# MAC-VO/MAC-VO

Hardware: AMD Instinct MI355X
Metric: stereo frames/sec at 640x480 (hot path: cost volume + lookup, keypoint selection, covariance, PGO) (higher is better)
Workload: dtype f32 via f16x2 (volume: fp32 operands row-scaled by powers of two and split into two fp16 pieces, three products, fp32 accumulate, scales undone exactly) + f32 (lookup/covariance) + f64 (PGO)

## Files before the change

mac-vo_amd/csrc/frontend_ops.hip:

```cpp
#include "common.h"
#include "randperm_dev.h"
#include "kp_draw_dev.h"
#include "match_cov_dev.h"
#include "pose_apply_dev.h"
#include "obs_filter_dev.h"
#include <math.h>

namespace {

__global__ __launch_bounds__(256) void frontend_epilogue_kernel(
    const float* __restrict__ flow, const float* __restrict__ logcov, int cov_is_log, int plane, float bl_fx,
    float bl_fx_sq, float* __restrict__ disparity, float* __restrict__ disparity_cov, float* __restrict__ depth,
    float* __restrict__ depth_cov, uint8_t* __restrict__ bad_mask, float* __restrict__ match_flow,
    float* __restrict__ match_cov) {
    MV_CHAIN_KERNEL_PRIO();
    const size_t lo = (size_t)blockIdx.y * plane;
    flow += 4 * lo; logcov += 4 * lo;
    if (disparity) disparity += lo;
    if (disparity_cov) disparity_cov += lo;
    if (depth) depth += lo;
    if (depth_cov) depth_cov += lo;
    if (bad_mask) bad_mask += lo;
    if (match_flow) match_flow += 2 * lo;
    if (match_cov) match_cov += 3 * lo;
// ... 224 lines not shown
    if (out_sdd) out_sdd[n] = depth_cov ? depth_cov[i] : -1.f;
    if (out_sigma) { out_sigma[3 * n] = match_cov_default; out_sigma[3 * n + 1] = match_cov_default; out_sigma[3 * n + 2] = 0.f; }
    const float pc[3] = {d, ((uf - cx) * d) / fx, ((vf - cy) * d) / fy};
    if (out_Tc) { out_Tc[3 * n] = pc[0]; out_Tc[3 * n + 1] = pc[1]; out_Tc[3 * n + 2] = pc[2]; }
    if (out_Tw) {
        const float q[4] = {pose[3], pose[4], pose[5], pose[6]};
        float r[3];
        quat_act_f32(q, pc, r);
        out_Tw[3 * n] = r[0] + pose[0]; out_Tw[3 * n + 1] = r[1] + pose[1]; out_Tw[3 * n + 2] = r[2] + pose[2];
    }
    if (out_color && image) {
        const size_t plane = (size_t)H * W;
#pragma unroll
        for (int c = 0; c < 3; ++c) {
            const float x = image[c * plane + i] * 255.f;
            out_color[3 * n + c] = (uint8_t)(int)x;
        }
    }
}

__global__ __launch_bounds__(256) void obs_filter_kernel(const uint8_t* __restrict__ inbound,
                                                         const double* __restrict__ cov1,
                                                         const double* __restrict__ cov2,
                                                         const float* __restrict__ vals, int flags,
                                                         float min_depth, float max_depth, int cap, mvLaneCounts cnt,
                                                         uint8_t* __restrict__ valid, int32_t* __restrict__ count) {
    obs_filter_body(inbound, cov1, cov2, vals, flags, min_depth, max_depth, cap, cnt.n[blockIdx.x], blockIdx.x, gridDim.x, valid, count);
}

struct DrawArgs {
    const int32_t* count;
    int count_stride;
    float nomatch_c;
    const uint32_t* state_in;
    uint32_t* state_out;
    int k;
    int32_t cov_mods;
    int64_t* out_perm;
    int32_t* out_live;
};
struct DrawLds {
    mvrp::Scratch s;
    int32_t head[mvrp::NBUCKET];
    int32_t out[mvrp::MAX_HEAD];
};
template <int PM, int MODEL = MV_COV_MATCH, bool MODS = false, bool NOMATCH = false>
__global__ __launch_bounds__(256) void backend_front_kernel(const int32_t* __restrict__ cand, size_t cand_lane_stride, const int64_t* __restrict__ perm,
                                                            PermArg pa, int cap, mvLaneCounts cnt, int64_t* out_uv, TrackArgs a, float fx, float fy,
                                                            float cx, float cy, float* pos_Tc, const float* depth_map0, const float* depth_map1,
                                                            double* out_cov0, double* out_cov1, mvMatchCovParams cp, DrawArgs da) {
    __shared__ __attribute__((aligned(16))) char draw_raw[PM == 2 ? sizeof(DrawLds) : PM == 4 ? sizeof(mvkp::Scratch) : 16];
    DrawLds& D = *reinterpret_cast<DrawLds*>(draw_raw);
    const int lane = threadIdx.x & 63;
    const int n = blockIdx.x * 4 + (threadIdx.x >> 6);
    const int set = blockIdx.y, pl = blockIdx.z;
    int N;
    if constexpr (PM == 2) {
        const int64_t n_cand = da.count[(size_t)pl * da.count_stride];
        const bool adv = blockIdx.x == 0 && blockIdx.y == 0;
        N = mv_randperm_head_wg(da.state_in + (size_t)pl * mvrp::MT_STRIDE, adv ? da.state_out + (size_t)pl * mvrp::MT_STRIDE : nullptr, n_cand, da.k,
                                D.out, D.s, D.head);
        __syncthreads();
        if (adv) {
            for (int i = threadIdx.x; i < N; i += 256) da.out_perm[(size_t)pl * cap + i] = D.out[i];
            if (threadIdx.x == 0) { da.out_live[2 * pl] = N; da.out_live[2 * pl + 1] = (int32_t)n_cand; }
        }
    } else if constexpr (PM == 3) {
        if (da.count) {
            const int c = da.count[(size_t)pl * da.count_stride];
            N = c < 0 ? 0 : (c > cap ? cap : c);
        } else {
            N = cnt.n[pl];
        }
        if (da.out_live && blockIdx.x == 0 && blockIdx.y == 0 && threadIdx.x == 0) { da.out_live[2 * pl] = N; da.out_live[2 * pl + 1] = N; }
    } else if constexpr (PM == 4) {
        N = cnt.n[pl];
        const bool adv = blockIdx.x == 0 && blockIdx.y == 0;
        mv_kp_random_wg(da.state_in + (size_t)pl * mvrp::MT_STRIDE, adv ? da.state_out + (size_t)pl * mvrp::MT_STRIDE : nullptr, da.k,
                        *reinterpret_cast<mvkp::Scratch*>(draw_raw));
    } else {
        N = cnt.n[pl];
    }
    if (n < N) {
        int u0, v0;
        if constexpr (PM <= 2) {
            const int32_t* cand_l = cand + (size_t)pl * cand_lane_stride;
            const long pi = PM == 2 ? (long)D.out[n] : PM == 1 ? (long)pa.idx[n] : (long)perm[(size_t)pl * cap + n];
            const int lin = cand_l[pi];
            u0 = lin % a.W;
            v0 = lin / a.W;
        } else if constexpr (PM == 3) {
            const int64_t* kp = perm + 2 * ((size_t)pl * cap + n);
            u0 = (int)kp[0];
            v0 = (int)kp[1];
        } else if constexpr (PM == 4) {
            mvkp::row_of(reinterpret_cast<mvkp::Scratch*>(draw_raw)->w, da.k, n, a.H, a.W, pa.idx[0], u0, v0);
        } else {
            mvkp::grid_row(mvkp::Grid{pa.idx[0], 0, pa.idx[1], pa.idx[2], pa.idx[3]}, n, u0, v0);
        }
        TrackArgs al = a;
        track_lane_offsets(al, pl, cap);
        const size_t ln = (size_t)pl * cap;
        float u, v, suu, svv, suv;
        if (set == 0) {
            if (lane == 0) {
                if (PM != 3 || out_uv != perm) {
                    out_uv[2 * (ln + n) + 0] = u0;
                    out_uv[2 * (ln + n) + 1] = v0;
                }
                kp_track_one(n, u0, v0, al.match_flow, al.match_cov, al.depth0, al.disp0, al.sdisp0, al.sdd0, al.depth1, al.disp1, al.sdisp1, al.sdd1,
                             al.H, al.W, al.edge, al.match_cov_default, al.out_kp0, al.out_kp1, al.out_inbound, al.out_vals, (size_t)gridDim.z * cap,
                             nullptr, nullptr);
                al.out_sigma0[3 * n + 2] = 0.f;
                const float uf = (float)u0, vf = (float)v0, d = al.out_vals[n];
                float* pt = pos_Tc + 3 * (ln + n);
                pt[0] = d;
                pt[1] = ((uf - cx) * d) / fx;
                pt[2] = ((vf - cy) * d) / fy;
// ... 178 lines not shown
}

int mv_backend_front(const mvKpSource& src, int lanes, int cap, const mvFrontMaps& m, const mvCovConfig& cv, const mvFrontTables& t, mvStream_t stream) {
    const mvMatchCovParams& cp = cv.cp;
    const int kind = src.kind, num_point = src.num_point;
    MV_CHECK_ARG(kind >= MV_KPSRC_PERM && kind <= MV_KPSRC_GRID && cv.edge >= 0);
    if (kind != MV_KPSRC_PERM) MV_CHECK_ARG(lanes >= 1 && lanes <= MV_MAX_LANES && cap >= 1 && num_point >= 0);
    if (kind == MV_KPSRC_DRAW) MV_CHECK_ARG(num_point <= cap && src.n_live_stride >= 1);
    if (kind >= MV_KPSRC_ROWS) MV_CHECK_ARG(src.mask_width >= 0);
    MV_CHECK_ARG(cv.model >= MV_COV_MATCH && cv.model <= MV_COV_NONE && mv_cov_modifiers_ok(cv.modifiers));
    MV_CHECK_ARG(cv.model != MV_COV_GMM || (m.f0.sdd && m.f1.sdd));
    const bool nomatch = (cv.nocov & MV_NOCOV_MATCH) != 0;
    MV_CHECK_ARG(!nomatch || (m.match_cov == nullptr && kind >= MV_KPSRC_ROWS));
    MV_CHECK_ARG(!(cv.nocov & MV_NOCOV_DEPTH) || (cv.model != MV_COV_GMM && !m.f0.sdd && !m.f1.sdd && !m.f0.sdisp && !m.f1.sdisp));
    MV_CHECK_ARG(cp.H > 0 && cp.W > 0 && cp.kernel_size >= 1 && (cp.kernel_size & 1) && cp.use_patch_var);
    if (cp.kernel_size > mvcov::MAX_K || (kind == MV_KPSRC_DRAW && num_point > mvrp::MAX_HEAD)) return MV_ERR_UNSUPPORTED;
    mvLaneCounts c{};
    int n_max = 0;
    if (kind == MV_KPSRC_PERM) {
        const int rc = check_lanes(lanes, src.n_live, cap, c, n_max);
        if (rc != MV_OK) return rc;
        if (n_max == 0) return MV_OK;
    }
    MV_CHECK_ARG(m.match_flow && m.f0.depth && m.f1.depth && t.kp0_uv && t.kp1 && t.inbound && t.vals && t.sigma0 && t.sigma1 && t.pos_Tc && t.cov0 &&
                 t.cov1);
    const TrackArgs ta{m.match_flow, m.match_cov, m.f0.depth, m.f0.disp, m.f0.sdisp, m.f0.sdd, m.f1.depth, m.f1.disp, m.f1.sdisp, m.f1.sdd, cp.H, cp.W,
                       cv.edge, cv.match_cov_default, t.kp0, t.kp1, t.inbound, t.vals, t.sigma0, t.sigma1};
    const int32_t* cand = nullptr;
    size_t cand_stride = 0;
    const int64_t* rows = nullptr;
    PermArg pa;
    pa.idx[0] = 0;
    DrawArgs da{};
    int pm;
    if (kind == MV_KPSRC_PERM) {
        MV_CHECK_ARG(src.cand && (src.perm_dev || src.perm_host));
        cand = src.cand;
        cand_stride = src.cand_lane_stride;
        if (src.perm_host && lanes == 1 && n_max <= 256) {
            for (int i = 0; i < n_max; ++i) {
                MV_CHECK_ARG(src.perm_host[i] >= 0 && src.perm_host[i] <= 0x7fffffffLL);
                pa.idx[i] = (int32_t)src.perm_host[i];
            }
            pm = 1;
        } else {
            MV_CHECK_ARG(src.perm_dev);
            rows = src.perm_dev;
            pm = 0;
        }
    } else if (kind == MV_KPSRC_DRAW) {
        MV_CHECK_ARG(src.cand && src.n_live_dev && src.state_in && src.state_out && src.state_in != src.state_out && src.out_perm && src.out_live);
        cand = src.cand;
        cand_stride = src.cand_lane_stride;
        n_max = num_point > 0 ? num_point : 1;
        da = DrawArgs{src.n_live_dev, src.n_live_stride, 0.f, src.state_in, src.state_out, num_point, 0, src.out_perm, src.out_live};
        pm = 2;
    } else if (kind == MV_KPSRC_ROWS) {
        MV_CHECK_ARG(src.rows && (src.n_live || (src.n_live_dev && src.n_live_stride >= 1)));
        da.out_live = src.out_live;
        if (src.n_live) {
            const int rc = check_lanes(lanes, src.n_live, cap, c, n_max);
            if (rc != MV_OK) return rc;
        } else {
            n_max = cap;
            da.count = src.n_live_dev;
            da.count_stride = src.n_live_stride;
        }
        if (n_max == 0) return MV_OK;
        rows = src.rows;
        pm = 3;
    } else if (kind == MV_KPSRC_RANDOM) {
        MV_CHECK_ARG(src.state_in && src.state_out && src.state_in != src.state_out && num_point >= 1 && num_point <= cap && cp.H > 2 * src.mask_width &&
                     cp.W > 2 * src.mask_width);
        if (num_point > mvkp::MAX_POINT) return MV_ERR_UNSUPPORTED;
        n_max = num_point;
        pa.idx[0] = src.mask_width;
        da.state_in = src.state_in;
        da.state_out = src.state_out;
        da.k = num_point;
        pm = 4;
    } else {
        mvkp::Grid g;
        n_max = mvkp::grid_of(cp.H, cp.W, src.mask_width, num_point, &g);
        MV_CHECK_ARG(n_max >= 1 && n_max <= cap);
        pa.idx[0] = g.cols; pa.idx[1] = g.sh; pa.idx[2] = g.sw; pa.idx[3] = g.mask;
        pm = 5;
    }
    if (pm >= 4)
        for (int l = 0; l < lanes; ++l) c.n[l] = n_max;
    const dim3 grid(mv_ceil_div(n_max, 4), 2, lanes);
    launch_backend_front_pm(pm, cv.model, cv.modifiers, nomatch, cv.model_match_cov_default, grid, (hipStream_t)stream, da, cand, cand_stride, rows, pa, cap, c, t.kp0_uv, ta, cp.fx, cp.fy, cp.cx,
                            cp.cy, t.pos_Tc, m.f0.depth, m.f1.depth, t.cov0, t.cov1, cp);
    return mv_launch_status();
}

extern "C" int mv_backend_front_lanes(const int32_t* cand, size_t cand_lane_stride, const int64_t* perm_dev, const int64_t* perm_host, int lanes,
                                      const int32_t* n_live, int cap, const float* match_flow, const float* match_cov, const float* depth0,
                                      const float* disp0, const float* sdisp0, const float* sdd0, const float* depth1, const float* disp1,
                                      const float* sdisp1, const float* sdd1, int edge, float match_cov_default, const mvMatchCovParams* cov_params,
                                      int64_t* out_kp0_uv, float* out_kp0, float* out_kp1, uint8_t* out_inbound, float* out_vals, float* out_sigma0,
                                      float* out_sigma1, float* out_pos_Tc, double* out_cov0, double* out_cov1, mvStream_t stream) {
    MV_CHECK_ARG(cov_params);
    mvKpSource src{};
    src.kind = MV_KPSRC_PERM;
    src.cand = cand; src.cand_lane_stride = cand_lane_stride; src.perm_dev = perm_dev; src.perm_host = perm_host; src.n_live = n_live;
    return mv_backend_front(src, lanes, cap, {match_flow, match_cov, {depth0, disp0, sdisp0, sdd0}, {depth1, disp1, sdisp1, sdd1}},
                            {MV_COV_MATCH, 0, *cov_params, edge, match_cov_default},
                            {out_kp0_uv, out_kp0, out_kp1, out_inbound, out_vals, out_sigma0, out_sigma1, out_pos_Tc, out_cov0, out_cov1}, stream);
}

extern "C" int mv_backend_front_draw_lanes(const int32_t* cand, size_t cand_lane_stride, const int32_t* count_dev, int count_stride, const uint32_t* state_in,
                                           uint32_t* state_out, int num_point, int lanes, int cap, const float* match_flow, const float* match_cov,
                                           const float* depth0, const float* disp0, const float* sdisp0, const float* sdd0, const float* depth1,
                                           const float* disp1, const float* sdisp1, const float* sdd1, int edge, float match_cov_default,
                                           const mvMatchCovParams* cov_params, int64_t* out_perm, int32_t* out_live, int64_t* out_kp0_uv, float* out_kp0,
                                           float* out_kp1, uint8_t* out_inbound, float* out_vals, float* out_sigma0, float* out_sigma1, float* out_pos_Tc,
                                           double* out_cov0, double* out_cov1, mvStream_t stream) {
    MV_CHECK_ARG(cov_params);
    mvKpSource src{};
    src.kind = MV_KPSRC_DRAW;
    src.cand = cand; src.cand_lane_stride = cand_lane_stride; src.n_live_dev = count_dev; src.n_live_stride = count_stride;
    src.state_in = state_in; src.state_out = state_out; src.num_point = num_point; src.out_perm = out_perm; src.out_live = out_live;
    return mv_backend_front(src, lanes, cap, {match_flow, match_cov, {depth0, disp0, sdisp0, sdd0}, {depth1, disp1, sdisp1, sdd1}},
                            {MV_COV_MATCH, 0, *cov_params, edge, match_cov_default},
                            {out_kp0_uv, out_kp0, out_kp1, out_inbound, out_vals, out_sigma0, out_sigma1, out_pos_Tc, out_cov0, out_cov1}, stream);
}

extern "C" int mv_kp_track(const int64_t* kp0_uv, int N, const float* match_flow, const float* match_cov,
                           const float* depth0, const float* disp0, const float* sdisp0, const float* sdd0,
                           const float* depth1, const float* disp1, const float* sdisp1, const float* sdd1, int H,
                           int W, int edge, float match_cov_default, float* out_kp0, float* out_kp1,
                           uint8_t* out_inbound, float* out_vals, float* out_sigma0, float* out_sigma1,
                           mvStream_t stream) {
    MV_CHECK_ARG(N >= 0);
    const int32_t n = N;
    return mv_kp_track_lanes(kp0_uv, 1, &n, N, match_flow, match_cov, depth0, disp0, sdisp0, sdd0, depth1, disp1, sdisp1,
                             sdd1, H, W, edge, match_cov_default, out_kp0, out_kp1, out_inbound, out_vals, out_sigma0,
                             out_sigma1, stream);
}

extern "C" int mv_backproject_lanes(const float* kp_uv, const float* depth_vals, int depth_stride, size_t depth_lane_stride,
                                    float fx, float fy, float cx, float cy, const float* pose, int lanes,
                                    const int32_t* n_live, int cap, float* pos_Tc, float* pos_Tw, double* rot,
// ... 78 lines not shown
```

mac-vo_amd/csrc/kp_select.hip:

```cpp
#include "common.h"
#include <math.h>

namespace {

#ifdef MV_KP_PROFILE
__device__ long long g_kp_stamps[16];
#define KP_STAMP(i) do { if (threadIdx.x == 0) g_kp_stamps[i] = wall_clock64(); } while (0)
#else
#define KP_STAMP(i)
#endif

constexpr int TILE_W = 64;
constexpr int TILE_H = 16;
constexpr int MAX_R = 7;
constexpr unsigned CAND_FLAG = 0x80000000u;

struct KpWs {
    unsigned long long* cand_bits;
    unsigned* rec_idx;
    float* rec_q;
    float* rec_d;
    int* counters;
    size_t lane_bytes;

    __device__ __forceinline__ KpWs lane(int l) const {
        const size_t o = (size_t)l * lane_bytes;
        return KpWs{(unsigned long long*)((char*)cand_bits + o), (unsigned*)((char*)rec_idx + o), (float*)((char*)rec_q + o),
                    (float*)((char*)rec_d + o), (int*)((char*)counters + o), lane_bytes};
    }
};

__device__ __forceinline__ float flow_quality(const float* __restrict__ fc, int plane, int idx) {
    const float c0 = fc[idx], c1 = fc[plane + idx], c2 = fc[2 * plane + idx];
    return (c0 + c1) - 2.f * c2;
}

__device__ __forceinline__ float nanmin(float a, float b) { return (a < b || a != a) ? a : b; }

template <bool FUSE>
__global__ __launch_bounds__(256) void kp_nms_kernel(const float* __restrict__ fc, const float* __restrict__ d0,
                                                      const float* __restrict__ d0c, const float* __restrict__ d1,
                                                      const float* __restrict__ d1c,
                                                      const uint8_t* __restrict__ mask_a,
                                                      const uint8_t* __restrict__ mask_b, mvKpSelectParams p,
                                                      KpWs ws_all, int words_per_row, mvEpiArgs ef) {
    MV_CHAIN_KERNEL_PRIO();
    const KpWs ws = ws_all.lane(blockIdx.z);
    {
        const size_t lp = (size_t)blockIdx.z * p.H * p.W;
        if (fc) fc += 3 * lp;
        if (d0) d0 += lp;
        if (d0c) d0c += lp;
        if (d1) d1 += lp;
        if (d1c) d1c += lp;
        if (mask_a) mask_a += lp;
        if (mask_b) mask_b += lp;
        if (FUSE) {
            ef.flow += 4 * lp; ef.logcov += 4 * lp;
            if (ef.disparity) ef.disparity += lp;
            if (ef.disparity_cov) ef.disparity_cov += lp;
            if (ef.depth) ef.depth += lp;
            if (ef.depth_cov) ef.depth_cov += lp;
            if (ef.bad_mask) ef.bad_mask += lp;
            if (ef.match_flow) ef.match_flow += 2 * lp;
            if (ef.match_cov) ef.match_cov += 3 * lp;
        }
    }
    __shared__ float tile[TILE_H + 2 * MAX_R][TILE_W + 2 * MAX_R + 1];
    __shared__ float hmin[TILE_H + 2 * MAX_R][TILE_W + 1];
    __shared__ int wg_count, wg_base;
    const int H = p.H, W = p.W, plane = H * W;
    const int r = p.kernel_size >> 1;
    const int x0 = blockIdx.x * TILE_W, y0 = blockIdx.y * TILE_H;
    const int tx = threadIdx.x, ty = threadIdx.y;
    const int tid = ty * 64 + tx;
    const bool mapping = p.mode == MV_KP_MAPPING;
    if (tid == 0) wg_count = 0;

    if (!mapping) {
        const int tw = TILE_W + 2 * r, th = TILE_H + 2 * r;
        constexpr int NST = ((TILE_W + 2 * MAX_R) * (TILE_H + 2 * MAX_R) + 255) / 256;
// ... 29 lines not shown
        for (int e = tid; e < th * TILE_W; e += 256) {
            const int ly = e >> 6, lx = e & 63;
            float m = tile[ly][lx];
            for (int dx = 1; dx <= 2 * r; ++dx) m = nanmin(m, tile[ly][lx + dx]);
            hmin[ly][lx] = m;
        }
    }
    __syncthreads();

    bool nms_px[TILE_H / 4];
    bool cand_px[TILE_H / 4];
    float q_px[TILE_H / 4];
    int my_nms = 0;
#pragma unroll
    for (int it = 0; it < TILE_H / 4; ++it) {
        const int ly = ty * (TILE_H / 4) + it;
        const int gx = x0 + tx, gy = y0 + ly;
        const bool inimg = gx < W && gy < H;
        const int idx = gy * W + gx;
        bool nms = false, cand = false;
        float q = 0.f;
        if (FUSE && inimg) mv_epilogue_pixel(ef, plane, idx);
        if (inimg) {
            const bool border = p.mask_width > 0 && gx >= p.mask_width && gx < W - p.mask_width &&
                                gy >= p.mask_width && gy < H - p.mask_width;
            if (mapping) {
                cand = border && (d0[idx] < p.max_depth) && (d0c[idx] < p.max_depth_cov);
            } else {
                q = tile[ly + r][tx + r];
                float m = hmin[ly][tx];
                for (int dy = 1; dy <= 2 * r; ++dy) m = nanmin(m, hmin[ly + dy][tx]);
                nms = (q == m);
                cand = nms && border;
                if (cand && p.mode == MV_KP_FULL) cand = (d0[idx] < p.max_depth) && (d1[idx] < p.max_depth);
            }
            if (cand && mask_a) cand = mask_a[idx] != 0;
            if (cand && mask_b) cand = mask_b[idx] != 0;
        }
        const unsigned long long cand_word = __ballot(cand);
        if (tx == 0 && gy < H) ws.cand_bits[(size_t)gy * words_per_row + blockIdx.x] = cand_word;
        nms_px[it] = nms;
        cand_px[it] = cand;
        q_px[it] = q;
        my_nms += nms;
    }
    if (mapping) return;

    int my_off = 0;
    if (my_nms) my_off = atomicAdd(&wg_count, my_nms);
    __syncthreads();
#ifdef MV_KP_FAKE_ATOMIC
    if (tid == 0) wg_base = (blockIdx.y * gridDim.x + blockIdx.x) * 16;
#else
    if (tid == 0) wg_base = wg_count ? atomicAdd(&ws.counters[0], wg_count) : 0;
#endif
    __syncthreads();
    int pos = wg_base + my_off;
#pragma unroll
    for (int it = 0; it < TILE_H / 4; ++it) {
        if (nms_px[it]) {
            const int gx = x0 + tx, gy = y0 + ty * (TILE_H / 4) + it;
            const int idx = gy * W + gx;
            ws.rec_idx[pos] = (unsigned)(((gy * words_per_row + blockIdx.x) << 6) | tx) | (cand_px[it] ? CAND_FLAG : 0u);
            if (p.mode == MV_KP_NODEPTH) {
                ws.rec_q[pos] = q_px[it];
            } else {
                ws.rec_q[pos] = fc ? flow_quality(fc, plane, idx) : 0.f;
                ws.rec_d[pos] = d0c[idx];
            }
            ++pos;
        }
    }
}

__device__ __forceinline__ unsigned float_key(float f) {
    if (f != f) return 0xFFFFFFFFu;
    const unsigned u = __float_as_uint(f);
    return (u & 0x80000000u) ? ~u : (u | 0x80000000u);
}
__device__ __forceinline__ float key_float(unsigned k) {
    const unsigned u = (k & 0x80000000u) ? (k & 0x7FFFFFFFu) : ~k;
    return __uint_as_float(u);
}

#ifndef MV_KP_FINISH_THREADS
#define MV_KP_FINISH_THREADS 1024
#endif

constexpr int RANK_CAP = 256;
constexpr unsigned NAN_KEY = 0xFFFFFFFFu;

template <int NT>
__device__ __forceinline__ int block_exclusive_scan(int v, int* wave_tot , int& total) {
    constexpr int NW = NT / 64;
    const int tid = threadIdx.x;
    int incl = v;
#pragma unroll
    for (int o = 1; o < 64; o <<= 1) {
        const int t = __shfl_up(incl, o, 64);
        if ((tid & 63) >= o) incl += t;
    }
    __syncthreads();
    if ((tid & 63) == 63) wave_tot[tid >> 6] = incl;
    __syncthreads();
    int off = 0;
    total = 0;
#pragma unroll
    for (int w = 0; w < NW; ++w) {
        const int t = wave_tot[w];
        if (w < (tid >> 6)) off += t;
        total += t;
    }
    return off + incl - v;
}

template <int NT, bool CACHED, int RPT, typename F>
__device__ __forceinline__ void for_each_key(const float* __restrict__ vals, int n, const unsigned (&keys)[RPT], F&& f) {
    const int tid = threadIdx.x;
    if (CACHED) {
        const int nr = (n + NT - 1) / NT;
#pragma unroll
        for (int r = 0; r < RPT; ++r)
            if (r < nr && r * NT + tid < n) f(keys[r]);
    } else {
        for (int i = tid; i < n; i += NT) f(float_key(vals[i]));
    }
}

struct MedianLds {
    unsigned hist[2048];
    unsigned lst[RANK_CAP];
    unsigned red_lo[16], red_hi[16];
    int red_cnt[16];
    int wave_tot[16];
    int sh[4];
    unsigned res;
};

template <int NT, bool CACHED, int RPT>
__device__ float block_nanmedian(const float* __restrict__ vals, int n, const unsigned (&keys)[RPT], MedianLds& L) {
    constexpr int NW = NT / 64, BPT = 2048 / NT;
    const int tid = threadIdx.x;
    unsigned lo = NAN_KEY, hi = 0u;
    int cnt = 0;
    for_each_key<NT, CACHED, RPT>(vals, n, keys, [&](unsigned k) {
        if (k != NAN_KEY) {
            lo = min(lo, k);
            hi = max(hi, k);
            ++cnt;
        }
    });
#pragma unroll
    for (int o = 32; o > 0; o >>= 1) {
        lo = min(lo, (unsigned)__shfl_xor((int)lo, o, 64));
        hi = max(hi, (unsigned)__shfl_xor((int)hi, o, 64));
        cnt += __shfl_xor(cnt, o, 64);
    }
    __syncthreads();
    if ((tid & 63) == 0) {
        L.red_lo[tid >> 6] = lo;
        L.red_hi[tid >> 6] = hi;
        L.red_cnt[tid >> 6] = cnt;
    }
    __syncthreads();
    cnt = 0;
#pragma unroll
    for (int w = 0; w < NW; ++w) {
        lo = min(lo, L.red_lo[w]);
        hi = max(hi, L.red_hi[w]);
        cnt += L.red_cnt[w];
    }
    if (cnt <= 0) return NAN;
    int k = (cnt - 1) >> 1;
    for (;;) {
        if (lo == hi) return key_float(lo);
        const unsigned span = hi - lo;
        const int s = max(0, 32 - __clz((int)span) - 11);
#pragma unroll
        for (int j = 0; j < BPT; ++j) L.hist[j * NT + tid] = 0;
        if (tid == 0) L.sh[3] = 0;
        __syncthreads();
        for_each_key<NT, CACHED, RPT>(vals, n, keys, [&](unsigned kk) {
            if (kk >= lo && kk <= hi) atomicAdd(&L.hist[(kk - lo) >> s], 1u);
        });
        __syncthreads();
        int c[BPT], sum = 0;
#pragma unroll
        for (int j = 0; j < BPT; ++j) {
            c[j] = (int)L.hist[tid * BPT + j];
            sum += c[j];
        }
        int total;
        const int excl = block_exclusive_scan<NT>(sum, L.wave_tot, total);
        if (excl <= k && k < excl + sum) {
            int before = excl;
#pragma unroll
            for (int j = 0; j < BPT; ++j) {
                if (k >= before && k < before + c[j]) {
                    L.sh[0] = tid * BPT + j;
                    L.sh[1] = c[j];
                    L.sh[2] = k - before;
                }
                before += c[j];
            }
        }
        __syncthreads();
        const unsigned b = (unsigned)L.sh[0];
        const int cb = L.sh[1];
        k = L.sh[2];
        const unsigned nlo = lo + (b << s);
        const unsigned w = s ? ((1u << s) - 1u) : 0u;
        const unsigned nhi = (hi - nlo < w) ? hi : nlo + w;
        if (cb <= RANK_CAP) {
            for_each_key<NT, CACHED, RPT>(vals, n, keys, [&](unsigned kk) {
                if (kk >= nlo && kk <= nhi) L.lst[atomicAdd(&L.sh[3], 1)] = kk;
            });
            __syncthreads();
            for (int i = tid; i < cb; i += NT) {
                const unsigned e = L.lst[i];
                int rank = 0;
                for (int j = 0; j < cb; ++j) {
                    const unsigned o = L.lst[j];
                    rank += (o < e) || (o == e && j < i);
                }
                if (rank == k) L.res = e;
            }
            __syncthreads();
            return key_float(L.res);
        }
        lo = nlo;
        hi = nhi;
        __syncthreads();
    }
}

template <int NT, bool FAST, int RPT, int WPT, bool USE_D>
__device__ __forceinline__ void kp_finish_body(const mvKpSelectParams& p, const KpWs& ws, int has_flow, int words_per_row,
                                               int32_t* __restrict__ out_cand, int32_t* __restrict__ out_count,
                                               float* __restrict__ out_stats, int n_rec, MedianLds& L,
                                               unsigned long long* lds_words) {
    constexpr int RD = USE_D ? RPT : 1;
    const int tid = threadIdx.x;
    const int H = p.H, W = p.W;
    const bool mapping = p.mode == MV_KP_MAPPING;
    const bool use_f = (p.mode == MV_KP_NODEPTH) || (p.mode == MV_KP_FULL && has_flow);
    const bool use_d = USE_D && (p.mode == MV_KP_FULL);
    const int n_words = H * words_per_row;

    unsigned kq[RPT], kd[RD], ridx[RPT];
    unsigned long long wreg[WPT];
    KP_STAMP(0);
    if (FAST) {
        const int cap = H * W;
#pragma unroll
        for (int r = 0; r < RPT; ++r) {
            const int i = min(r * NT + tid, cap - 1);
            ridx[r] = mapping ? 0u : ws.rec_idx[i];
            kq[r] = use_f ? __float_as_uint(ws.rec_q[i]) : 0u;
            if (USE_D) kd[r] = use_d ? __float_as_uint(ws.rec_d[i]) : 0u;
        }
#pragma unroll
        for (int j = 0; j < WPT; ++j) {
            const int w = j * NT + tid;
            wreg[j] = w < n_words ? ws.cand_bits[w] : 0ull;
        }
#pragma unroll
        for (int r = 0; r < RPT; ++r) {
            const bool live = r * NT + tid < n_rec;
            ridx[r] = live ? ridx[r] : 0u;
            kq[r] = live ? float_key(__uint_as_float(kq[r])) : NAN_KEY;
            if (USE_D) kd[r] = live ? float_key(__uint_as_float(kd[r])) : NAN_KEY;
        }
    }

    float med_f = NAN, thr_f = INFINITY, med_d = NAN, thr_d = INFINITY;
    KP_STAMP(1);
    if (use_f) {
        med_f = block_nanmedian<NT, FAST, RPT>(ws.rec_q, n_rec, kq, L);
        const float prod = med_f * 1.5f;
        thr_f = (prod < p.max_match_cov) ? prod : p.max_match_cov;
    }
    if (use_d) {
        med_d = block_nanmedian<NT, FAST, RD>(ws.rec_d, n_rec, kd, L);
        const float prod = med_d * 1.5f;
        thr_d = (prod < p.max_depth_cov) ? prod : p.max_depth_cov;
    }

    KP_STAMP(2);
    const int per = (n_words + NT - 1) / NT;
    unsigned long long cw[WPT];
    if (FAST) {
        constexpr int NPASS = WPT > 5 * 1024 / NT ? 8 : 2;
        constexpr int TPP = NT / NPASS;
        unsigned fail = 0;
        if (!mapping) {
            const int nr = (n_rec + NT - 1) / NT;
#pragma unroll
            for (int r = 0; r < RPT; ++r) {
                if (r < nr && (ridx[r] & CAND_FLAG)) {
                    bool ok = true;
                    if (use_f) ok = key_float(kq[r]) < thr_f;
                    if (USE_D) { if (ok && use_d) ok = key_float(kd[USE_D ? r : 0]) < thr_d; }
                    if (!ok) fail |= 1u << r;
                }
            }
        }
#pragma unroll
        for (int i = 0; i < WPT; ++i) cw[i] = 0ull;
#pragma unroll 1
        for (int h = 0; h < NPASS; ++h) {
            const int wlo = h * TPP * per, whi = min(wlo + TPP * per, n_words);
#pragma unroll
            for (int j = 0; j < WPT; ++j) {
                const int w = j * NT + tid;
                if (w >= wlo && w < whi) lds_words[w - wlo] = wreg[j];
            }
            __syncthreads();
            if (fail) {
#pragma unroll
                for (int r = 0; r < RPT; ++r) {
                    const int w = (int)((ridx[r] & ~CAND_FLAG) >> 6);
                    if (((fail >> r) & 1u) && w >= wlo && w < whi) atomicAnd(&lds_words[w - wlo], ~(1ull << (ridx[r] & 63)));
                }
            }
            __syncthreads();
            if (tid / TPP == h) {
#pragma unroll
                for (int i = 0; i < WPT; ++i) {
                    const int w = tid * per + i;
                    if (i < per && w < whi) cw[i] = lds_words[w - wlo];
                }
            }
            __syncthreads();
        }
    } else if (!mapping) {
        for (int i = tid; i < n_rec; i += NT) {
            const unsigned ri = ws.rec_idx[i];
            if (ri & CAND_FLAG) {
                bool ok = true;
                if (use_f) ok = ws.rec_q[i] < thr_f;
                if (ok && use_d) ok = ws.rec_d[i] < thr_d;
                if (!ok) atomicAnd(&ws.cand_bits[(ri & ~CAND_FLAG) >> 6], ~(1ull << (ri & 63)));
            }
        }
        __threadfence();
        __syncthreads();
    }

    KP_STAMP(3);
    const int w_begin = min(tid * per, n_words), w_end = min(w_begin + per, n_words);
    int cnt = 0;
    if (FAST) {
#pragma unroll
        for (int i = 0; i < WPT; ++i) cnt += __popcll(cw[i]);
    } else {
        for (int w = w_begin; w < w_end; ++w)
            cnt += __popcll(__hip_atomic_load(&ws.cand_bits[w], __ATOMIC_RELAXED, __HIP_MEMORY_SCOPE_AGENT));
    }
    int total;
    int pos = block_exclusive_scan<NT>(cnt, L.wave_tot, total);
    KP_STAMP(4);
    auto emit = [&](unsigned long long bits, int w) {
        const int row = w / words_per_row, col0 = (w - row * words_per_row) * 64;
        while (bits) {
            const int bpos = __ffsll((long long)bits) - 1;
            bits &= bits - 1;
            out_cand[pos++] = row * W + col0 + bpos;
        }
    };
    if (FAST) {
#pragma unroll
        for (int i = 0; i < WPT; ++i)
            if (cw[i]) emit(cw[i], w_begin + i);
    } else {
        for (int w = w_begin; w < w_end; ++w)
            emit(__hip_atomic_load(&ws.cand_bits[w], __ATOMIC_RELAXED, __HIP_MEMORY_SCOPE_AGENT), w);
    }
    KP_STAMP(5);
    if (tid == 0) {
        ws.counters[0] = 0;
        out_count[0] = total;
        out_count[1] = n_rec;
        out_count[2] = 0;
        out_count[3] = 0;
        out_stats[0] = med_f;
        out_stats[1] = thr_f;
        out_stats[2] = med_d;
        out_stats[3] = thr_d;
    }
}

template <int NT, int RPT, int WPT, bool USE_D>
__global__ __launch_bounds__(NT) void kp_finish_kernel(mvKpSelectParams p, KpWs ws_all, int has_flow, int words_per_row,
                                                        int32_t* __restrict__ out_cand, int32_t* __restrict__ out_count,
                                                        float* __restrict__ out_stats) {
    __shared__ MedianLds L;
    extern __shared__ unsigned long long lds_words[];
    MV_CHAIN_KERNEL_PRIO();
    const KpWs ws = ws_all.lane(blockIdx.x);
    out_cand += (size_t)blockIdx.x * p.H * p.W;
    out_count += 4 * blockIdx.x;
    out_stats += 4 * blockIdx.x;
    const int n_rec = p.mode == MV_KP_MAPPING ? 0 : ws.counters[0];
    if (n_rec <= RPT * NT && p.H * words_per_row <= WPT * NT)
        kp_finish_body<NT, true, RPT, WPT, USE_D>(p, ws, has_flow, words_per_row, out_cand, out_count, out_stats, n_rec, L,
                                                  lds_words);
    else
        kp_finish_body<NT, false, RPT, WPT, USE_D>(p, ws, has_flow, words_per_row, out_cand, out_count, out_stats, n_rec, L,
                                                   lds_words);
}

template <int NT, int RPT, int WPT, bool USE_D>
static int launch_finish(const mvKpSelectParams& p, const KpWs& ws, int has_flow, int wpr, int32_t* out_cand,
                         int32_t* out_count, float* out_stats, int lanes, hipStream_t s) {
    const size_t dyn = (size_t)WPT * (NT / (WPT > 5 * 1024 / NT ? 8 : 2)) * sizeof(unsigned long long);
    hipLaunchKernelGGL((kp_finish_kernel<NT, RPT, WPT, USE_D>), dim3(lanes), dim3(NT), dyn, s, p, ws, has_flow, wpr, out_cand,
                       out_count, out_stats);
    return MV_OK;
}

__global__ __launch_bounds__(1024) void kp_map_scan_kernel(const unsigned long long* __restrict__ cand_bits, int n_words,
                                                            int* __restrict__ word_off, int32_t* __restrict__ out_count,
                                                            float* __restrict__ out_stats) {
    __shared__ int wave_tot[16];
    const int tid = threadIdx.x;
    const int per = (n_words + 1023) / 1024;
    const int w_begin = min(tid * per, n_words), w_end = min(w_begin + per, n_words);
    int cnt = 0;
    for (int w = w_begin; w < w_end; ++w) cnt += __popcll(cand_bits[w]);
    int total;
    int pos = block_exclusive_scan<1024>(cnt, wave_tot, total);
    for (int w = w_begin; w < w_end; ++w) {
        word_off[w] = pos;
        pos += __popcll(cand_bits[w]);
    }
    if (tid == 0) {
        out_count[0] = total;
        out_count[1] = out_count[2] = out_count[3] = 0;
        out_stats[0] = NAN;
        out_stats[1] = INFINITY;
        out_stats[2] = NAN;
        out_stats[3] = INFINITY;
    }
}

__global__ __launch_bounds__(256) void kp_map_emit_kernel(const unsigned long long* __restrict__ cand_bits,
                                                           const int* __restrict__ word_off, int n_words, int words_per_row,
                                                           int W, int32_t* __restrict__ out_cand) {
    const int w = blockIdx.x * 4 + (threadIdx.x >> 6);
    if (w >= n_words) return;
    const int lane = threadIdx.x & 63;
    const unsigned long long bits = cand_bits[w];
    if ((bits >> lane) & 1ull) {
        const int rank = __popcll(bits & ((1ull << lane) - 1ull));
        const int row = w / words_per_row, col0 = (w - row * words_per_row) * 64;
        out_cand[word_off[w] + rank] = row * W + col0 + lane;
    }
}

__global__ void kp_gather_kernel(const int32_t* __restrict__ cand, const int64_t* __restrict__ perm, mvLaneCounts cnt,
                                 int cap, size_t cand_lane_stride, int W, int64_t* __restrict__ out_uv) {
    const int i = blockIdx.x * blockDim.x + threadIdx.x;
    const int n_sel = cnt.n[blockIdx.y];
    cand += (size_t)blockIdx.y * cand_lane_stride;
    perm += (size_t)blockIdx.y * cap;
    out_uv += 2 * (size_t)blockIdx.y * cap;
    if (i < n_sel) {
        const int lin = cand[perm[i]];
        out_uv[2 * i + 0] = lin % W;
        out_uv[2 * i + 1] = lin / W;
    }
}

inline size_t align_up(size_t v, size_t a) { return (v + a - 1) / a * a; }

}

extern "C" size_t mv_kp_select_workspace_bytes(int H, int W) {
    if (H <= 0 || W <= 0) return 0;
    const size_t words = (size_t)H * mv_ceil_div(W, 64);
    return align_up(words * 8, 256) + 3 * align_up((size_t)H * W * 4, 256) + 256;
}

static int kp_select_impl(const float* flow_cov, const float* depth0, const float* depth0_cov, const float* depth1,
                          const float* depth1_cov, const uint8_t* mask_a, const uint8_t* mask_b, const mvKpSelectParams* params,
                          void* workspace, size_t workspace_bytes, int32_t* out_cand, int32_t* out_count, float* out_stats,
                          int lanes, mvStream_t stream, const mvEpiArgs* fuse) {
    MV_CHECK_ARG(lanes >= 1 && lanes <= MV_MAX_LANES);
    MV_CHECK_ARG(params && workspace && out_cand && out_count && out_stats);
    const mvKpSelectParams p = *params;
    MV_CHECK_ARG(p.H > 0 && p.W > 0 && p.mask_width >= 0);
    if (p.mode == MV_KP_NODEPTH) {
        MV_CHECK_ARG(flow_cov);
    } else if (p.mode == MV_KP_FULL) {
        MV_CHECK_ARG(depth0 && depth0_cov && depth1 && depth1_cov);
    } else if (p.mode == MV_KP_MAPPING) {
        MV_CHECK_ARG(depth0 && depth0_cov);
    } else {
        return MV_ERR_INVALID_ARG;
    }
    if (p.mode != MV_KP_MAPPING) {
        MV_CHECK_ARG(p.kernel_size >= 1 && (p.kernel_size & 1));
        if (p.kernel_size > 2 * MAX_R + 1) return MV_ERR_UNSUPPORTED;
    }
    const size_t lane_bytes = mv_kp_select_workspace_bytes(p.H, p.W);
    if (workspace_bytes < lane_bytes * (size_t)lanes) return MV_ERR_WORKSPACE;
    if (((uintptr_t)workspace & 7) != 0) return MV_ERR_INVALID_ARG;
    if (p.mode == MV_KP_MAPPING && lanes != 1) return MV_ERR_UNSUPPORTED;

    const int wpr = mv_ceil_div(p.W, 64);
    const size_t words = (size_t)p.H * wpr;
    const size_t plane_bytes = align_up((size_t)p.H * p.W * 4, 256);
    char* base = (char*)workspace;
    KpWs ws;
    ws.cand_bits = (unsigned long long*)base;
    base += align_up(words * 8, 256);
    ws.rec_idx = (unsigned*)base;
    base += plane_bytes;
    ws.rec_q = (float*)base;
    base += plane_bytes;
    ws.rec_d = (float*)base;
    base += plane_bytes;
    ws.counters = (int*)base;
    ws.lane_bytes = lane_bytes;

    hipStream_t s = (hipStream_t)stream;
    dim3 grid(wpr, mv_ceil_div(p.H, TILE_H), lanes), block(64, 4);
    if (fuse)
        hipLaunchKernelGGL(kp_nms_kernel<true>, grid, block, 0, s, flow_cov, depth0, depth0_cov, depth1, depth1_cov, mask_a,
                           mask_b, p, ws, wpr, *fuse);
    else
        hipLaunchKernelGGL(kp_nms_kernel<false>, grid, block, 0, s, flow_cov, depth0, depth0_cov, depth1, depth1_cov, mask_a,
                           mask_b, p, ws, wpr, mvEpiArgs{});
    if (p.mode == MV_KP_MAPPING) {
        const int n_words = p.H * wpr;
        int* word_off = (int*)ws.rec_idx;
        hipLaunchKernelGGL(kp_map_scan_kernel, dim3(1), dim3(1024), 0, s, ws.cand_bits, n_words, word_off, out_count, out_stats);
        hipLaunchKernelGGL(kp_map_emit_kernel, dim3(mv_ceil_div(n_words, 4)), dim3(256), 0, s, ws.cand_bits, word_off, n_words,
                           wpr, p.W, out_cand);
        return mv_launch_status();
    }
    const bool big = (size_t)p.H * wpr > 5 * (size_t)1024;
    const bool full = p.mode == MV_KP_FULL;
    int rc;
    static int small_nt = -1;
    if (small_nt < 0) { const char* e = getenv("MV_KP_FINISH_SMALL_NT"); small_nt = (e && atoi(e) == 512) ? 512 : 1024; }
    if (big) rc = full ? launch_finish<1024, 24, 15, true>(p, ws, flow_cov ? 1 : 0, wpr, out_cand, out_count, out_stats, lanes, s)
                       : launch_finish<1024, 24, 15, false>(p, ws, flow_cov ? 1 : 0, wpr, out_cand, out_count, out_stats, lanes, s);
    else if (small_nt == 512)
        rc = full ? launch_finish<512, 16, 10, true>(p, ws, flow_cov ? 1 : 0, wpr, out_cand, out_count, out_stats, lanes, s)
                  : launch_finish<512, 16, 10, false>(p, ws, flow_cov ? 1 : 0, wpr, out_cand, out_count, out_stats, lanes, s);
    else rc = full ? launch_finish<1024, 16, 5, true>(p, ws, flow_cov ? 1 : 0, wpr, out_cand, out_count, out_stats, lanes, s)
                   : launch_finish<1024, 16, 5, false>(p, ws, flow_cov ? 1 : 0, wpr, out_cand, out_count, out_stats, lanes, s);
    if (rc != MV_OK) return rc;
    return mv_launch_status();
}

extern "C" int mv_kp_select_lanes(const float* flow_cov, const float* depth0, const float* depth0_cov,
                                  const float* depth1, const float* depth1_cov, const uint8_t* mask_a,
                                  const uint8_t* mask_b, const mvKpSelectParams* params, void* workspace,
                                  size_t workspace_bytes, int32_t* out_cand, int32_t* out_count, float* out_stats,
                                  int lanes, mvStream_t stream) {
    return kp_select_impl(flow_cov, depth0, depth0_cov, depth1, depth1_cov, mask_a, mask_b, params, workspace, workspace_bytes,
                          out_cand, out_count, out_stats, lanes, stream, nullptr);
}

extern "C" int mv_frontend_epilogue_select_lanes(const float* flow, const float* logcov, int cov_is_log, float bl_fx,
                                                 float bl_fx_sq, float* disparity, float* disparity_cov, float* depth,
                                                 float* depth_cov, uint8_t* bad_mask, float* match_flow, float* match_cov,
                                                 const uint8_t* mask_a, const uint8_t* mask_b, const mvKpSelectParams* params,
                                                 void* workspace, size_t workspace_bytes, int32_t* out_cand,
                                                 int32_t* out_count, float* out_stats, int lanes, mvStream_t stream) {
    MV_CHECK_ARG(flow && logcov && params && match_cov);
    if (params->mode != MV_KP_NODEPTH) return MV_ERR_UNSUPPORTED;
    const mvEpiArgs ef{flow, logcov, cov_is_log, bl_fx, bl_fx_sq, disparity, disparity_cov, depth, depth_cov, match_flow, match_cov,
                       bad_mask};
// ... 37 lines not shown
```

mac-vo_amd/csrc/randperm_dev.h:

```cpp
#pragma once
#include <stdint.h>

#if defined(__HIPCC__)
#define MV_RP_FN __host__ __device__ __forceinline__
#else
#define MV_RP_FN inline
#endif

namespace mvrp {

constexpr int MT_N = 624;
constexpr int MT_STRIDE = 640;
constexpr int MAX_HEAD = 512;
constexpr int NBUCKET = 1024;

struct Scratch {
    uint32_t mt[2][MT_N];
    int32_t t[MAX_HEAD], nxt[MAX_HEAD], ptr[MAX_HEAD], hit[MAX_HEAD];
};

MV_RP_FN uint32_t mt_f(uint32_t a, uint32_t b) {
    const uint32_t y = (a & 0x80000000u) | (b & 0x7fffffffu);
    return (y >> 1) ^ ((b & 1u) ? 0x9908b0dfu : 0u);
}
// ... 87 lines not shown

template <typename T>
MV_RP_FN void phase_emit(const Scratch& s, const Plan& pl, T* out, int tid, int nt) {
    for (int i = tid; i < pl.m; i += nt) {
        const int32_t h = s.hit[i];
        out[i] = (T)(h == -2 ? root_of(s, i) : (h >= 0 ? root_of(s, h) : s.t[i]));
    }
}

}

#if defined(__HIPCC__)
template <typename T>
__device__ __forceinline__ int mv_randperm_head_wg(const uint32_t* __restrict__ state_in, uint32_t* state_out, int64_t n, int k, T* out, mvrp::Scratch& s,
                                                   int32_t* head) {
    using namespace mvrp;
    const int tid = threadIdx.x, nt = blockDim.x;
    const Plan pl = plan_of(n, k);
    phase_clear(head, tid, nt);
    if (pl.advance > 0 || state_out) {
        for (int i = tid; i < MT_N; i += nt) s.mt[0][i] = state_in[i];
        int pos = (int)state_in[MT_N];
        __syncthreads();
        int cur = 0;
        int64_t produced = 0;
        const int64_t total = state_out ? pl.advance : (int64_t)pl.swaps;
        int64_t rem = total;
        while (rem > 0) {
            if (pos == MT_N) {
                phase_step(s.mt[cur], s.mt[cur ^ 1], tid, nt);
                __syncthreads();
                cur ^= 1;
                pos = 0;
            }
            const int take = (int)(rem < MT_N - pos ? rem : MT_N - pos);
            if (produced < pl.swaps) phase_draws(s.mt[cur], pos, take, produced, pl, s.t, tid, nt);
            pos += take;
            produced += take;
            rem -= take;
        }
        if (state_out) {
            for (int i = tid; i < MT_N; i += nt) state_out[i] = s.mt[cur][i];
            if (tid == 0) state_out[MT_N] = (uint32_t)pos;
        }
    }
    __syncthreads();
    phase_insert(s, head, pl, tid, nt);
    __syncthreads();
    phase_link(s, head, pl, tid, nt);
    __syncthreads();
    phase_emit(s, pl, out, tid, nt);
    return pl.m;
}
#endif
```

Baseline: 7183.

## Shard keypoint record counters and split randperm state advance into dedicated block

Keypoint selection now spreads its global atomic record counter across eight padded shards, each with its own region, so fewer workgroups contend on one atomic. The finish kernel rebuilds a prefix map to read the sharded records. In the draw path, the long Mersenne-Twister state advance moves into an extra leading block, so the compute blocks only produce the permutation head and do not wait on the full advance. The cost is an index remap on every record read, extra workspace, and one more block in the grid.

New measurement: 7170. No clear change (-0.2%).

```diff
diff --git a/mac-vo_amd/csrc/frontend_ops.hip b/mac-vo_amd/csrc/frontend_ops.hip
--- a/mac-vo_amd/csrc/frontend_ops.hip
+++ b/mac-vo_amd/csrc/frontend_ops.hip
@@ -300,18 +300,20 @@
     __shared__ __attribute__((aligned(16))) char draw_raw[PM == 2 ? sizeof(DrawLds) : PM == 4 ? sizeof(mvkp::Scratch) : 16];
     DrawLds& D = *reinterpret_cast<DrawLds*>(draw_raw);
     const int lane = threadIdx.x & 63;
-    const int n = blockIdx.x * 4 + (threadIdx.x >> 6);
+    const int n = ((int)blockIdx.x - (PM == 2 ? 1 : 0)) * 4 + (threadIdx.x >> 6);
     const int set = blockIdx.y, pl = blockIdx.z;
     int N;
     if constexpr (PM == 2) {
         const int64_t n_cand = da.count[(size_t)pl * da.count_stride];
-        const bool adv = blockIdx.x == 0 && blockIdx.y == 0;
-        N = mv_randperm_head_wg(da.state_in + (size_t)pl * mvrp::MT_STRIDE, adv ? da.state_out + (size_t)pl * mvrp::MT_STRIDE : nullptr, n_cand, da.k,
-                                D.out, D.s, D.head);
+        const bool adv = blockIdx.x == 0;
+        if (adv && blockIdx.y != 0) return;
+        N = mv_randperm_head_wg(da.state_in + (size_t)pl * mvrp::MT_STRIDE, nullptr, n_cand, da.k, D.out, D.s, D.head);
         __syncthreads();
         if (adv) {
             for (int i = threadIdx.x; i < N; i += 256) da.out_perm[(size_t)pl * cap + i] = D.out[i];
             if (threadIdx.x == 0) { da.out_live[2 * pl] = N; da.out_live[2 * pl + 1] = (int32_t)n_cand; }
+            mv_randperm_advance_wg(da.state_in + (size_t)pl * mvrp::MT_STRIDE, da.state_out + (size_t)pl * mvrp::MT_STRIDE, n_cand, D.s);
+            return;
         }
     } else if constexpr (PM == 3) {
         if (da.count) {
@@ -596,7 +598,7 @@
         MV_CHECK_ARG(src.cand && src.n_live_dev && src.state_in && src.state_out && src.state_in != src.state_out && src.out_perm && src.out_live);
         cand = src.cand;
         cand_stride = src.cand_lane_stride;
-        n_max = num_point > 0 ? num_point : 1;
+        n_max = num_point;
         da = DrawArgs{src.n_live_dev, src.n_live_stride, 0.f, src.state_in, src.state_out, num_point, 0, src.out_perm, src.out_live};
         pm = 2;
     } else if (kind == MV_KPSRC_ROWS) {
@@ -632,7 +634,7 @@
     }
     if (pm >= 4)
         for (int l = 0; l < lanes; ++l) c.n[l] = n_max;
-    const dim3 grid(mv_ceil_div(n_max, 4), 2, lanes);
+    const dim3 grid(mv_ceil_div(n_max, 4) + (pm == 2 ? 1 : 0), 2, lanes);
     launch_backend_front_pm(pm, cv.model, cv.modifiers, nomatch, cv.model_match_cov_default, grid, (hipStream_t)stream, da, cand, cand_stride, rows, pa, cap, c, t.kp0_uv, ta, cp.fx, cp.fy, cp.cx,
                             cp.cy, t.pos_Tc, m.f0.depth, m.f1.depth, t.cov0, t.cov1, cp);
     return mv_launch_status();
diff --git a/mac-vo_amd/csrc/kp_select.hip b/mac-vo_amd/csrc/kp_select.hip
--- a/mac-vo_amd/csrc/kp_select.hip
+++ b/mac-vo_amd/csrc/kp_select.hip
@@ -14,6 +14,8 @@
 constexpr int TILE_H = 16;
 constexpr int MAX_R = 7;
 constexpr unsigned CAND_FLAG = 0x80000000u;
+constexpr int REC_SHARDS = 8;
+constexpr int REC_CTR_STRIDE = 32;
 
 struct KpWs {
     unsigned long long* cand_bits;
@@ -21,12 +23,13 @@
     float* rec_q;
     float* rec_d;
     int* counters;
+    int rec_region;
     size_t lane_bytes;
 
     __device__ __forceinline__ KpWs lane(int l) const {
         const size_t o = (size_t)l * lane_bytes;
         return KpWs{(unsigned long long*)((char*)cand_bits + o), (unsigned*)((char*)rec_idx + o), (float*)((char*)rec_q + o),
-                    (float*)((char*)rec_d + o), (int*)((char*)counters + o), lane_bytes};
+                    (float*)((char*)rec_d + o), (int*)((char*)counters + o), rec_region, lane_bytes};
     }
 };
 
@@ -162,7 +165,10 @@
 #ifdef MV_KP_FAKE_ATOMIC
     if (tid == 0) wg_base = (blockIdx.y * gridDim.x + blockIdx.x) * 16;
 #else
-    if (tid == 0) wg_base = wg_count ? atomicAdd(&ws.counters[0], wg_count) : 0;
+    if (tid == 0) {
+        const int shard = (blockIdx.y * gridDim.x + blockIdx.x) & (REC_SHARDS - 1);
+        wg_base = shard * ws.rec_region + (wg_count ? atomicAdd(&ws.counters[shard * REC_CTR_STRIDE], wg_count) : 0);
+    }
 #endif
     __syncthreads();
     int pos = wg_base + my_off;
@@ -224,8 +230,20 @@
     return off + incl - v;
 }
 
+struct RecMap {
+    int pre[REC_SHARDS];
+    int n_rec, region;
+    __device__ __forceinline__ int at(int i) const {
+        int a = i;
+#pragma unroll
+        for (int k = 1; k < REC_SHARDS; ++k)
+            if (i >= pre[k]) a = k * region + (i - pre[k]);
+        return a;
+    }
+};
+
 template <int NT, bool CACHED, int RPT, typename F>
-__device__ __forceinline__ void for_each_key(const float* __restrict__ vals, int n, const unsigned (&keys)[RPT], F&& f) {
+__device__ __forceinline__ void for_each_key(const float* __restrict__ vals, const RecMap& rm, int n, const unsigned (&keys)[RPT], F&& f) {
     const int tid = threadIdx.x;
     if (CACHED) {
         const int nr = (n + NT - 1) / NT;
@@ -233,7 +251,7 @@
         for (int r = 0; r < RPT; ++r)
             if (r < nr && r * NT + tid < n) f(keys[r]);
     } else {
-        for (int i = tid; i < n; i += NT) f(float_key(vals[i]));
+        for (int i = tid; i < n; i += NT) f(float_key(vals[rm.at(i)]));
     }
 }
 
@@ -248,12 +266,12 @@
 };
 
 template <int NT, bool CACHED, int RPT>
-__device__ float block_nanmedian(const float* __restrict__ vals, int n, const unsigned (&keys)[RPT], MedianLds& L) {
+__device__ float block_nanmedian(const float* __restrict__ vals, const RecMap& rm, int n, const unsigned (&keys)[RPT], MedianLds& L) {
     constexpr int NW = NT / 64, BPT = 2048 / NT;
     const int tid = threadIdx.x;
     unsigned lo = NAN_KEY, hi = 0u;
     int cnt = 0;
-    for_each_key<NT, CACHED, RPT>(vals, n, keys, [&](unsigned k) {
+    for_each_key<NT, CACHED, RPT>(vals, rm, n, keys, [&](unsigned k) {
         if (k != NAN_KEY) {
             lo = min(lo, k);
             hi = max(hi, k);
@@ -290,7 +308,7 @@
         for (int j = 0; j < BPT; ++j) L.hist[j * NT + tid] = 0;
         if (tid == 0) L.sh[3] = 0;
         __syncthreads();
-        for_each_key<NT, CACHED, RPT>(vals, n, keys, [&](unsigned kk) {
+        for_each_key<NT, CACHED, RPT>(vals, rm, n, keys, [&](unsigned kk) {
             if (kk >= lo && kk <= hi) atomicAdd(&L.hist[(kk - lo) >> s], 1u);
         });
         __syncthreads();
@@ -322,7 +340,7 @@
         const unsigned w = s ? ((1u << s) - 1u) : 0u;
         const unsigned nhi = (hi - nlo < w) ? hi : nlo + w;
         if (cb <= RANK_CAP) {
-            for_each_key<NT, CACHED, RPT>(vals, n, keys, [&](unsigned kk) {
+            for_each_key<NT, CACHED, RPT>(vals, rm, n, keys, [&](unsigned kk) {
                 if (kk >= nlo && kk <= nhi) L.lst[atomicAdd(&L.sh[3], 1)] = kk;
             });
             __syncthreads();
@@ -347,7 +365,7 @@
 template <int NT, bool FAST, int RPT, int WPT, bool USE_D>
 __device__ __forceinline__ void kp_finish_body(const mvKpSelectParams& p, const KpWs& ws, int has_flow, int words_per_row,
                                                int32_t* __restrict__ out_cand, int32_t* __restrict__ out_count,
-                                               float* __restrict__ out_stats, int n_rec, MedianLds& L,
+                                               float* __restrict__ out_stats, const RecMap& rm, MedianLds& L,
                                                unsigned long long* lds_words) {
     constexpr int RD = USE_D ? RPT : 1;
     const int tid = threadIdx.x;
@@ -356,15 +374,16 @@
     const bool use_f = (p.mode == MV_KP_NODEPTH) || (p.mode == MV_KP_FULL && has_flow);
     const bool use_d = USE_D && (p.mode == MV_KP_FULL);
     const int n_words = H * words_per_row;
+    const int n_rec = rm.n_rec;
 
     unsigned kq[RPT], kd[RD], ridx[RPT];
     unsigned long long wreg[WPT];
     KP_STAMP(0);
     if (FAST) {
-        const int cap = H * W;
 #pragma unroll
         for (int r = 0; r < RPT; ++r) {
-            const int i = min(r * NT + tid, cap - 1);
+            const bool live = r * NT + tid < n_rec;
+            const int i = live ? rm.at(r * NT + tid) : 0;
             ridx[r] = mapping ? 0u : ws.rec_idx[i];
             kq[r] = use_f ? __float_as_uint(ws.rec_q[i]) : 0u;
             if (USE_D) kd[r] = use_d ? __float_as_uint(ws.rec_d[i]) : 0u;
@@ -386,12 +405,12 @@
     float med_f = NAN, thr_f = INFINITY, med_d = NAN, thr_d = INFINITY;
     KP_STAMP(1);
     if (use_f) {
-        med_f = block_nanmedian<NT, FAST, RPT>(ws.rec_q, n_rec, kq, L);
+        med_f = block_nanmedian<NT, FAST, RPT>(ws.rec_q, rm, n_rec, kq, L);
         const float prod = med_f * 1.5f;
         thr_f = (prod < p.max_match_cov) ? prod : p.max_match_cov;
     }
     if (use_d) {
-        med_d = block_nanmedian<NT, FAST, RD>(ws.rec_d, n_rec, kd, L);
+        med_d = block_nanmedian<NT, FAST, RD>(ws.rec_d, rm, n_rec, kd, L);
         const float prod = med_d * 1.5f;
         thr_d = (prod < p.max_depth_cov) ? prod : p.max_depth_cov;
     }
@@ -444,7 +463,8 @@
             __syncthreads();
         }
     } else if (!mapping) {
-        for (int i = tid; i < n_rec; i += NT) {
+        for (int j = tid; j < n_rec; j += NT) {
+            const int i = rm.at(j);
             const unsigned ri = ws.rec_idx[i];
             if (ri & CAND_FLAG) {
                 bool ok = true;
@@ -487,8 +507,8 @@
             emit(__hip_atomic_load(&ws.cand_bits[w], __ATOMIC_RELAXED, __HIP_MEMORY_SCOPE_AGENT), w);
     }
     KP_STAMP(5);
+    if (tid < REC_SHARDS) ws.counters[tid * REC_CTR_STRIDE] = 0;
     if (tid == 0) {
-        ws.counters[0] = 0;
         out_count[0] = total;
         out_count[1] = n_rec;
         out_count[2] = 0;
@@ -511,12 +531,20 @@
     out_cand += (size_t)blockIdx.x * p.H * p.W;
     out_count += 4 * blockIdx.x;
     out_stats += 4 * blockIdx.x;
-    const int n_rec = p.mode == MV_KP_MAPPING ? 0 : ws.counters[0];
+    RecMap rm;
+    rm.region = ws.rec_region;
+    int n_rec = 0;
+#pragma unroll
+    for (int k = 0; k < REC_SHARDS; ++k) {
+        rm.pre[k] = n_rec;
+        n_rec += p.mode == MV_KP_MAPPING ? 0 : ws.counters[k * REC_CTR_STRIDE];
+    }
+    rm.n_rec = n_rec;
     if (n_rec <= RPT * NT && p.H * words_per_row <= WPT * NT)
-        kp_finish_body<NT, true, RPT, WPT, USE_D>(p, ws, has_flow, words_per_row, out_cand, out_count, out_stats, n_rec, L,
+        kp_finish_body<NT, true, RPT, WPT, USE_D>(p, ws, has_flow, words_per_row, out_cand, out_count, out_stats, rm, L,
                                                   lds_words);
     else
-        kp_finish_body<NT, false, RPT, WPT, USE_D>(p, ws, has_flow, words_per_row, out_cand, out_count, out_stats, n_rec, L,
+        kp_finish_body<NT, false, RPT, WPT, USE_D>(p, ws, has_flow, words_per_row, out_cand, out_count, out_stats, rm, L,
                                                    lds_words);
 }
 
@@ -586,10 +614,19 @@
 
 }
 
+static size_t rec_region_of(int H, int W) {
+    const size_t tiles = (size_t)mv_ceil_div(W, TILE_W) * mv_ceil_div(H, TILE_H);
+    return (tiles + REC_SHARDS - 1) / REC_SHARDS * (TILE_W * TILE_H);
+}
+static size_t rec_array_bytes(int H, int W) {
+    const size_t rec = REC_SHARDS * rec_region_of(H, W), plane = (size_t)H * W;
+    return align_up((rec > plane ? rec : plane) * 4, 256);
+}
+
 extern "C" size_t mv_kp_select_workspace_bytes(int H, int W) {
     if (H <= 0 || W <= 0) return 0;
     const size_t words = (size_t)H * mv_ceil_div(W, 64);
-    return align_up(words * 8, 256) + 3 * align_up((size_t)H * W * 4, 256) + 256;
+    return align_up(words * 8, 256) + 3 * rec_array_bytes(H, W) + REC_SHARDS * REC_CTR_STRIDE * sizeof(int);
 }
 
 static int kp_select_impl(const float* flow_cov, const float* depth0, const float* depth0_cov, const float* depth1,
@@ -620,7 +657,7 @@
 
     const int wpr = mv_ceil_div(p.W, 64);
     const size_t words = (size_t)p.H * wpr;
-    const size_t plane_bytes = align_up((size_t)p.H * p.W * 4, 256);
+    const size_t plane_bytes = rec_array_bytes(p.H, p.W);
     char* base = (char*)workspace;
     KpWs ws;
     ws.cand_bits = (unsigned long long*)base;
@@ -632,6 +669,7 @@
     ws.rec_d = (float*)base;
     base += plane_bytes;
     ws.counters = (int*)base;
+    ws.rec_region = (int)rec_region_of(p.H, p.W);
     ws.lane_bytes = lane_bytes;
 
     hipStream_t s = (hipStream_t)stream;
diff --git a/mac-vo_amd/csrc/randperm_dev.h b/mac-vo_amd/csrc/randperm_dev.h
--- a/mac-vo_amd/csrc/randperm_dev.h
+++ b/mac-vo_amd/csrc/randperm_dev.h
@@ -163,4 +163,28 @@
     phase_emit(s, pl, out, tid, nt);
     return pl.m;
 }
+
+__device__ __forceinline__ void mv_randperm_advance_wg(const uint32_t* __restrict__ state_in, uint32_t* state_out, int64_t n, mvrp::Scratch& s) {
+    using namespace mvrp;
+    const int tid = threadIdx.x, nt = blockDim.x;
+    __syncthreads();
+    for (int i = tid; i < MT_N; i += nt) s.mt[0][i] = state_in[i];
+    int pos = (int)state_in[MT_N];
+    __syncthreads();
+    int cur = 0;
+    int64_t rem = plan_of(n, 0).advance;
+    while (rem > 0) {
+        if (pos == MT_N) {
+            phase_step(s.mt[cur], s.mt[cur ^ 1], tid, nt);
+            __syncthreads();
+            cur ^= 1;
+            pos = 0;
+        }
+        const int take = (int)(rem < MT_N - pos ? rem : MT_N - pos);
+        pos += take;
+        rem -= take;
+    }
+    for (int i = tid; i < MT_N; i += nt) state_out[i] = s.mt[cur][i];
+    if (tid == 0) state_out[MT_N] = (uint32_t)pos;
+}
 #endif
```
